# xavi-pinsach/kzg-grandsums-study

Hardware: AMD Instinct MI355X
Metric: grand-sum proofs/sec + MSM G1-adds/sec at n=2^20, 1/2/4/8 MI355X (higher is better)
Workload: dtype u32 limbs (BN254 Fr/Fq Montgomery: 8 x 32-bit; MSM buckets 9 x 29-bit), int VALU; 1 GPU; grandsum prover, n=2^20, k=1, no selectors, inputs resident in HBM; nbits=20, npols=1, selectors=False, parallelism=replicas x1, inflight_per_gpu=4, srs_power=20, srs_points_resident=2097151

## Files before the change

kzg-grandsums-study_amd/csrc/ntt.hip:

```cpp
#include <algorithm>
#include <cstdlib>
#include <map>
#include <mutex>
#include <type_traits>
#include <utility>

#include "fr29.hpp"
#include "kernels.hpp"

namespace kgs {

__device__ __forceinline__ uint32_t bitrev(uint32_t x, int bits) {
  return __builtin_bitreverse32(x) >> (32 - bits);
}

#ifndef KGS_NTT_CANON
__device__ __forceinline__ void bfly_dif(fr& x0, fr& x1, const uint32_t* w, bool tw) {
  const fr a = x0, b = x1;
  x0 = fr::add_lazy(a, b);
  x1 = tw ? fr::mul_nored(fr::sub_2p(a, b), fr::load(w)) : fr::sub_lazy(a, b);
}
__device__ __forceinline__ void bfly_dit(fr& x0, fr& x1, const uint32_t* w, bool tw) {
  const fr a = x0;
  const fr b = tw ? fr::mul_nored(x1, fr::load(w)) : x1;
  x0 = fr::add_lazy(a, b);
  x1 = fr::sub_lazy(a, b);
}
__device__ __forceinline__ fr canon_out(const fr& x) { return x.canon(); }
#else
__device__ __forceinline__ void bfly_dif(fr& x0, fr& x1, const uint32_t* w, bool tw) {
  const fr a = x0, b = x1;
  x0 = a + b;
  fr diff = a - b;
  if (tw) diff = diff * fr::load(w);
  x1 = diff;
}
__device__ __forceinline__ void bfly_dit(fr& x0, fr& x1, const uint32_t* w, bool tw) {
  const fr a = x0;
  fr b = x1;
  if (tw) b = b * fr::load(w);
  x0 = a + b;
  x1 = a - b;
}
__device__ __forceinline__ fr canon_out(const fr& x) { return x; }
#endif


template <int K>
__global__ void __launch_bounds__(256) k_ntt_dif_pass(uint32_t* __restrict__ data,
                                                      const uint32_t* __restrict__ in, uint64_t in_len,
                                                      const uint32_t* __restrict__ pre,
                                                      const uint32_t* __restrict__ tw, int logM, int logm,
                                                      int s0) {
  KGS_AUX_PRIO();
  const uint64_t m = 1ull << logm;
  const uint64_t ngroups = m >> K;
  const uint64_t g = (uint64_t)blockIdx.x * blockDim.x + threadIdx.x;
  if (g >= ngroups) return;
  const int logd = logm - s0 - K;
  const uint64_t d = 1ull << logd;
  const uint64_t lo = g & (d - 1), hi = g >> logd;
  const uint64_t base = (hi << (logd + K)) + lo;
  fr x[1 << K];
#pragma unroll
  for (int r = 0; r < (1 << K); r++) {
    uint64_t idx = base + ((uint64_t)r << logd);
    if (in) {
      if (idx < in_len) {
        x[r] = fr::load(in + 8 * idx);
        if (pre) x[r] = x[r] * fr::load(pre + 8 * idx);
      } else {
        x[r] = fr::zero();
      }
    } else {
      x[r] = fr::load(data + 8 * idx);
    }
  }
#pragma unroll
  for (int k = 0; k < K; k++) {
    const int s = s0 + k;
    const int logh = logm - s - 1;
    const int dist = 1 << (K - 1 - k);
    const uint64_t twbase = 1ull << logh;
#pragma unroll
    for (int j = 0; j < (1 << (K - 1)); j++) {
      const int r = ((j / dist) * 2 * dist) + (j % dist);
      const uint64_t t = lo + ((uint64_t)(j % dist) << logd);
      bfly_dif(x[r], x[r + dist], tw + 8 * (twbase + t), t != 0);
    }
  }
#pragma unroll
  for (int r = 0; r < (1 << K); r++) canon_out(x[r]).store(data + 8 * (base + ((uint64_t)r << logd)));
}

template <int K>
__global__ void __launch_bounds__(256) k_ntt_dit_pass(uint32_t* __restrict__ data,
                                                      const uint32_t* __restrict__ in, int in_bitrev,
                                                      const uint32_t* __restrict__ tw, int logM, int logm,
                                                      int s0, const uint32_t* __restrict__ post,
                                                      const uint32_t* __restrict__ post_s) {
  KGS_AUX_PRIO();
  const uint64_t m = 1ull << logm;
  const uint64_t ngroups = m >> K;
  const uint64_t g = (uint64_t)blockIdx.x * blockDim.x + threadIdx.x;
  if (g >= ngroups) return;
  const int logd = s0;
  const uint64_t d = 1ull << logd;
  const uint64_t lo = g & (d - 1), hi = g >> logd;
  const uint64_t base = (hi << (logd + K)) + lo;
  fr x[1 << K];
#pragma unroll
  for (int r = 0; r < (1 << K); r++) {
    uint64_t idx = base + ((uint64_t)r << logd);
    if (in) {
      uint64_t src = in_bitrev ? idx : (uint64_t)bitrev((uint32_t)idx, logm);
      x[r] = fr::load(in + 8 * src);
    } else {
      x[r] = fr::load(data + 8 * idx);
    }
  }
#pragma unroll
  for (int k = 0; k < K; k++) {
    const int s = s0 + k;
    const int dist = 1 << k;
    const uint64_t twbase = 1ull << s;
#pragma unroll
    for (int j = 0; j < (1 << (K - 1)); j++) {
      const int r = ((j / dist) * 2 * dist) + (j % dist);
      const uint64_t t = lo + ((uint64_t)(j % dist) << logd);
      bfly_dit(x[r], x[r + dist], tw + 8 * (twbase + t), t != 0);
    }
  }
  fr ps;
  if (post_s) ps = fr::load(post_s);
#pragma unroll
  for (int r = 0; r < (1 << K); r++) {
    uint64_t idx = base + ((uint64_t)r << logd);
    fr y = x[r];
    if (post) y = y * fr::load(post + 8 * idx);
    if (post_s) y = y * ps;
    canon_out(y).store(data + 8 * idx);
  }
}

static inline unsigned nblocks(uint64_t work, unsigned bs = 256) { return (unsigned)((work + bs - 1) / bs); }

#ifndef KGS_NTT_ELOG
#define KGS_NTT_ELOG 11
#endif
constexpr int NTT_ELOG = KGS_NTT_ELOG;
constexpr int LDS_ELEMS = 1 << NTT_ELOG;
constexpr int LDS_NT = LDS_ELEMS / 8;

__device__ __forceinline__ void lds_map(uint32_t e, int K, int logd, int lblog, uint32_t& j, uint32_t& cl) {
  if (logd >= lblog) {
    j = e >> lblog;
    cl = e & ((1u << lblog) - 1);
  } else {
    const uint32_t lo = e & ((1u << logd) - 1);
    j = (e >> logd) & ((1u << K) - 1);
    cl = ((e >> (logd + K)) << logd) | lo;
  }
}

__device__ __forceinline__ uint32_t lds_idx(uint32_t col, uint32_t j, int K, int logd) {
  const uint32_t lo = col & ((1u << logd) - 1), hi = col >> logd;
  return (hi << (logd + K)) | (j << logd) | lo;
}

#ifndef KGS_NTT_LDS_AOS
__device__ __forceinline__ uint32_t lds_swz(uint32_t e) { return e ^ ((e >> 4) & 15u) ^ ((e >> 8) & 15u); }
__device__ __forceinline__ fr lds_ld(const uint32_t* lds, uint32_t e) {
  e = lds_swz(e);
  const uint4 a = reinterpret_cast<const uint4*>(lds)[e];
  const uint4 b = reinterpret_cast<const uint4*>(lds + 4 * LDS_ELEMS)[e];
  fr r;
  r.v[0] = a.x; r.v[1] = a.y; r.v[2] = a.z; r.v[3] = a.w;
  r.v[4] = b.x; r.v[5] = b.y; r.v[6] = b.z; r.v[7] = b.w;
  return r;
}
__device__ __forceinline__ void lds_st(uint32_t* lds, uint32_t e, const fr& x) {
  e = lds_swz(e);
  reinterpret_cast<uint4*>(lds)[e] = make_uint4(x.v[0], x.v[1], x.v[2], x.v[3]);
  reinterpret_cast<uint4*>(lds + 4 * LDS_ELEMS)[e] = make_uint4(x.v[4], x.v[5], x.v[6], x.v[7]);
}
#else
__device__ __forceinline__ fr lds_ld(const uint32_t* lds, uint32_t e) { return fr::load(lds + 8 * e); }
__device__ __forceinline__ void lds_st(uint32_t* lds, uint32_t e, const fr& x) { x.store(lds + 8 * e); }
#endif

struct ntt_io {
  uint32_t* data;
  const uint32_t* in;
  uint64_t in_len;
  int in_bitrev;
  const uint32_t* pre;
  const uint32_t* post;
  const uint32_t* post_s;
  int logm;
  const uint32_t* pre29;
  const uint32_t* post29;
  const uint32_t* post_s29;
};

template <bool DIT, bool T29>
__device__ __forceinline__ fr ntt_load(const ntt_io& io, uint64_t idx) {
  if (!io.in) return fr::load(io.data + 8 * idx);
  if (DIT) return fr::load(io.in + 8 * (io.in_bitrev ? idx : (uint64_t)bitrev((uint32_t)idx, io.logm)));
  if (idx >= io.in_len) return fr::zero();
  fr x = fr::load(io.in + 8 * idx);
  if (io.pre) x = T29 ? mul29(x, w29_load(io.pre29 + TW29_WORDS * idx)) : x * fr::load(io.pre + 8 * idx);
  return x;
}
template <bool T29>
__device__ __forceinline__ void ntt_store(const ntt_io& io, uint64_t idx, fr y) {
  if (io.post) y = T29 ? mul29(y, w29_load(io.post29 + TW29_WORDS * idx)) : y * fr::load(io.post + 8 * idx);
  if (io.post_s) y = T29 ? mul29(y, w29_load(io.post_s29)) : y * fr::load(io.post_s);
  canon_out(y).store(io.data + 8 * idx);
}

template <typename TW>
__device__ __forceinline__ TW tw_load(const uint32_t* tw, uint32_t idx);
template <>
__device__ __forceinline__ fr tw_load<fr>(const uint32_t* tw, uint32_t idx) { return fr::load(tw + 8 * idx); }
template <>
__device__ __forceinline__ W29 tw_load<W29>(const uint32_t* tw, uint32_t idx) {
  return w29_load(tw + TW29_WORDS * idx);
}
__device__ __forceinline__ void mul_tw_x2(const fr& a, const fr& wa, const fr& b, const fr& wb, fr& ra, fr& rb) {
  fr::mul_nored_x2(a, wa, b, wb, ra, rb);
}
__device__ __forceinline__ void mul_tw_x2(const fr& a, const W29& wa, const fr& b, const W29& wb, fr& ra, fr& rb) {
  ra = mul29(a, wa);
  rb = mul29(b, wb);
}

template <typename F, int... I>
__device__ __forceinline__ void static_for_impl(F&& f, std::integer_sequence<int, I...>) {
  (f(std::integral_constant<int, I>{}), ...);
}
template <int N, typename F>
__device__ __forceinline__ void static_for(F&& f) {
  static_for_impl(f, std::make_integer_sequence<int, N>{});
}

__device__ __forceinline__ void bfly_pair_triv(fr* x, int r0, int r1, int dist) {
  const fr a0 = x[r0], b0 = x[r0 + dist], a1 = x[r1], b1 = x[r1 + dist];
  x[r0] = fr::add_lazy(a0, b0);
  x[r0 + dist] = fr::sub_lazy(a0, b0);
  x[r1] = fr::add_lazy(a1, b1);
  x[r1 + dist] = fr::sub_lazy(a1, b1);
}
template <bool DIT, typename TW>
__device__ __forceinline__ void bfly_pair_x2(fr* x, int r0, int r1, int dist, const TW& w0, const TW& w1) {
  if (DIT) {
    fr b0, b1;
    mul_tw_x2(x[r0 + dist], w0, x[r1 + dist], w1, b0, b1);
    const fr a0 = x[r0], a1 = x[r1];
    x[r0] = fr::add_lazy(a0, b0);
    x[r0 + dist] = fr::sub_lazy(a0, b0);
    x[r1] = fr::add_lazy(a1, b1);
    x[r1 + dist] = fr::sub_lazy(a1, b1);
  } else {
    const fr d0 = fr::sub_2p(x[r0], x[r0 + dist]), d1 = fr::sub_2p(x[r1], x[r1 + dist]);
    x[r0] = fr::add_lazy(x[r0], x[r0 + dist]);
    x[r1] = fr::add_lazy(x[r1], x[r1 + dist]);
    mul_tw_x2(d0, w0, d1, w1, x[r0 + dist], x[r1 + dist]);
  }
}
template <int R, bool DIT, bool GIN, bool GOUT, bool PF, typename TW>
__device__ __forceinline__ void lds_round(uint32_t* lds, const uint32_t* __restrict__ tw, const ntt_io& io, uint32_t cl,
                                          uint32_t col, uint32_t jb, uint32_t js, int K, int logd, int lb, int kp0) {
  constexpr bool T29 = std::is_same<TW, W29>::value;
  fr x[1 << R];
  if (GIN && !DIT && io.in && io.pre && R >= 2) {
    static_for<(1 << R) / 2>([&](auto rc) {
      constexpr int r = 2 * decltype(rc)::value;
      const uint32_t i0 = lds_idx(col, jb + js * r, K, logd), i1 = lds_idx(col, jb + js * (r + 1), K, logd);
      if (__builtin_expect(__all(i0 >= io.in_len && i1 >= io.in_len), 0)) {
        x[r] = fr::zero();
        x[r + 1] = fr::zero();
        return;
      }
      const fr a0 = i0 < io.in_len ? fr::load(io.in + 8 * i0) : fr::zero();
      const fr a1 = i1 < io.in_len ? fr::load(io.in + 8 * i1) : fr::zero();
      if constexpr (T29) {
        x[r] = mul29(a0, w29_load(io.pre29 + TW29_WORDS * i0));
        x[r + 1] = mul29(a1, w29_load(io.pre29 + TW29_WORDS * i1));
      } else {
        fr::mul_nored_x2(a0, fr::load(io.pre + 8 * i0), a1, fr::load(io.pre + 8 * i1), x[r], x[r + 1]);
      }
    });
  } else {
    static_for<(1 << R)>([&](auto rc) {
      constexpr int r = decltype(rc)::value;
      x[r] = GIN ? ntt_load<DIT, T29>(io, lds_idx(col, jb + js * r, K, logd)) : lds_ld(lds, (jb + js * r) * lb + cl);
    });
  }
#ifdef KGS_NTT_SINGLE
  constexpr bool kPairs = T29;
#else
  constexpr bool kPairs = true;
#endif
  if constexpr (R >= 2 && kPairs) {
    constexpr int half = 1 << (R - 2);
    constexpr int NSTEP = R * half;
    uint32_t tw0[NSTEP], tw1[NSTEP];
    bool triv[NSTEP];
#pragma unroll
    for (int k = 0; k < R; k++) {
      const int kp = kp0 + k;
      const int logh = DIT ? logd + kp : logd + K - 1 - kp;
      const int dist = DIT ? 1 << k : 1 << (R - 1 - k);
      const uint32_t hm = (1u << logh) - 1;
#pragma unroll
      for (int qa = 0; qa < half; qa++) {
        const int r0 = ((qa / dist) * 2 * dist) + (qa % dist), r1 = (((qa + half) / dist) * 2 * dist) + ((qa + half) % dist);
        const uint32_t t0 = lds_idx(col, jb + js * r0, K, logd) & hm, t1 = lds_idx(col, jb + js * r1, K, logd) & hm;
        tw0[k * half + qa] = hm + 1 + t0;
        tw1[k * half + qa] = hm + 1 + t1;
        triv[k * half + qa] = __all(t0 == 0 && t1 == 0);
      }
    }
    TW wa, wb;
    if (PF) {
      wa = tw_load<TW>(tw, tw0[0]);
      wb = tw_load<TW>(tw, tw1[0]);
    }
    static_for<NSTEP>([&](auto stc) {
      constexpr int st = decltype(stc)::value;
      constexpr int k = st / half, qa = st % half;
      constexpr int dist = DIT ? 1 << k : 1 << (R - 1 - k);
      constexpr int r0 = ((qa / dist) * 2 * dist) + (qa % dist), r1 = (((qa + half) / dist) * 2 * dist) + ((qa + half) % dist);
      if (PF) {
        constexpr int nx = st + 1 < NSTEP ? st + 1 : st;
        const TW na = tw_load<TW>(tw, tw0[nx]), nb = tw_load<TW>(tw, tw1[nx]);
        if (triv[st])
          bfly_pair_triv(x, r0, r1, dist);
        else
          bfly_pair_x2<DIT>(x, r0, r1, dist, wa, wb);
        wa = na;
        wb = nb;
      } else if (triv[st]) {
        bfly_pair_triv(x, r0, r1, dist);
      } else {
        bfly_pair_x2<DIT>(x, r0, r1, dist, tw_load<TW>(tw, tw0[st]), tw_load<TW>(tw, tw1[st]));
      }
    });
  } else {
    static_assert(sizeof(TW) == sizeof(fr), "the single-butterfly path reads 8 x 32-bit twiddles only");
#pragma unroll
    for (int k = 0; k < R; k++) {
      const int kp = kp0 + k;
      const int logh = DIT ? logd + kp : logd + K - 1 - kp;
      const int dist = DIT ? 1 << k : 1 << (R - 1 - k);
#pragma unroll
      for (int q = 0; q < (1 << (R - 1)); q++) {
        const int r = ((q / dist) * 2 * dist) + (q % dist);
        const uint32_t idx = lds_idx(col, jb + js * r, K, logd);
        const uint32_t t = idx & ((1u << logh) - 1);
        const uint32_t* w = tw + 8 * ((1u << logh) + t);
        if (DIT)
          bfly_dit(x[r], x[r + dist], w, t != 0);
        else
          bfly_dif(x[r], x[r + dist], w, t != 0);
      }
    }
  }
  if (GOUT && R >= 2) {
    if (io.post) {
      static_for<(1 << R) / 2>([&](auto rc) {
        constexpr int r = 2 * decltype(rc)::value;
        const uint32_t i0 = lds_idx(col, jb + js * r, K, logd), i1 = lds_idx(col, jb + js * (r + 1), K, logd);
        if constexpr (T29) {
          x[r] = mul29(x[r], w29_load(io.post29 + TW29_WORDS * i0));
          x[r + 1] = mul29(x[r + 1], w29_load(io.post29 + TW29_WORDS * i1));
        } else {
          fr::mul_nored_x2_ip(x[r], fr::load(io.post + 8 * i0), x[r + 1], fr::load(io.post + 8 * i1));
        }
      });
    }
    if (io.post_s) {
      if constexpr (T29) {
        const W29 ps = w29_load(io.post_s29);
        static_for<(1 << R)>([&](auto rc) {
          constexpr int r = decltype(rc)::value;
          x[r] = mul29(x[r], ps);
        });
      } else {
        const fr ps = fr::load(io.post_s);
#pragma unroll
        for (int r = 0; r < (1 << R); r += 2) fr::mul_nored_x2_ip(x[r], ps, x[r + 1], ps);
      }
    }
#pragma unroll
    for (int r = 0; r < (1 << R); r++) canon_out(x[r]).store(io.data + 8 * lds_idx(col, jb + js * r, K, logd));
    return;
  }
#pragma unroll
  for (int r = 0; r < (1 << R); r++) {
    if (GOUT)
      ntt_store<T29>(io, lds_idx(col, jb + js * r, K, logd), x[r]);
    else
      lds_st(lds, (jb + js * r) * lb + cl, x[r]);
  }
}

template <int R, bool DIT, bool GIN, bool GOUT, bool PF, typename TW>
__device__ __forceinline__ void lds_round_all(uint32_t* lds, const uint32_t* __restrict__ tw, const ntt_io& io,
                                              uint32_t col0, int K, int logd, int lblog, int b0) {
  const int kp0 = DIT ? b0 : K - b0 - R;
  for (uint32_t g = threadIdx.x; g < (LDS_ELEMS >> R); g += LDS_NT) {
    const uint32_t cl = g & ((1u << lblog) - 1), jq = g >> lblog;
    const uint32_t jb = (jq & ((1u << b0) - 1)) | ((jq >> b0) << (b0 + R));
    lds_round<R, DIT, GIN, GOUT, PF, TW>(lds, tw, io, cl, col0 + cl, jb, 1u << b0, K, logd, 1 << lblog, kp0);
  }
}

#ifndef KGS_NTT_PF3
#define KGS_NTT_PF3 0
#endif
template <int K1, int K2, int K3, int K4, bool DIT, bool DIRECT, int WV, bool T29>
__global__ void __launch_bounds__(LDS_NT) __attribute__((amdgpu_waves_per_eu(WV, WV)))
k_ntt_lds_pass(ntt_io io, const uint32_t* __restrict__ tw, int s0) {
  using TW = typename std::conditional<T29, W29, fr>::type;
  KGS_AUX_PRIO();
  constexpr int K = K1 + K2 + K3 + K4;
  static_assert(K4 == 0 || K3 > 0, "rounds are filled in order");
  constexpr int LBLOG = NTT_ELOG - K;
  constexpr int LB = 1 << LBLOG;
  uint32_t* lds;
  if constexpr (WV >= 3) {
    extern __shared__ __attribute__((aligned(16))) uint32_t lds_dyn[];
    lds = lds_dyn;
  } else {
    __shared__ __attribute__((aligned(16))) uint32_t lds_tile[LDS_ELEMS * 8];
    lds = lds_tile;
  }
  const int logd = DIT ? s0 : io.logm - s0 - K;
  const uint32_t col0 = blockIdx.x * LB;
  if (!DIRECT) {
    for (uint32_t e = threadIdx.x; e < LDS_ELEMS; e += LDS_NT) {
      uint32_t j, cl;
      lds_map(e, K, logd, LBLOG, j, cl);
      lds_st(lds, j * LB + cl, ntt_load<DIT, T29>(io, lds_idx(col0 + cl, j, K, logd)));
    }
    __syncthreads();
  }
  constexpr bool PF = WV < 3 || KGS_NTT_PF3;
  lds_round_all<K1, DIT, DIRECT, false, PF, TW>(lds, tw, io, col0, K, logd, LBLOG, DIT ? 0 : K - K1);
  __syncthreads();
  if constexpr (K4 > 0) {
    lds_round_all<K2, DIT, false, false, PF, TW>(lds, tw, io, col0, K, logd, LBLOG, DIT ? K1 : K3 + K4);
    __syncthreads();
    lds_round_all<K3, DIT, false, false, PF, TW>(lds, tw, io, col0, K, logd, LBLOG, DIT ? K1 + K2 : K4);
    __syncthreads();
    lds_round_all<K4, DIT, false, DIRECT, PF, TW>(lds, tw, io, col0, K, logd, LBLOG, DIT ? K1 + K2 + K3 : 0);
  } else if constexpr (K3 > 0) {
    lds_round_all<K2, DIT, false, false, PF, TW>(lds, tw, io, col0, K, logd, LBLOG, DIT ? K1 : K3);
    __syncthreads();
    lds_round_all<K3, DIT, false, DIRECT, PF, TW>(lds, tw, io, col0, K, logd, LBLOG, DIT ? K1 + K2 : 0);
  } else {
    lds_round_all<K2, DIT, false, DIRECT, PF, TW>(lds, tw, io, col0, K, logd, LBLOG, DIT ? K1 : 0);
  }
  if (!DIRECT) {
    __syncthreads();
    for (uint32_t e = threadIdx.x; e < LDS_ELEMS; e += LDS_NT) {
      uint32_t j, cl;
      lds_map(e, K, logd, LBLOG, j, cl);
      ntt_store<T29>(io, lds_idx(col0 + cl, j, K, logd), lds_ld(lds, j * LB + cl));
    }
  }
}

thread_local bool g_ntt_coresident = false;

struct Tw29Entry {
  uint64_t count;
  const uint32_t* twin;
};
static std::mutex g_tw29_mu;
static std::map<const uint32_t*, Tw29Entry> g_tw29;
void ntt_register_tw29(const uint32_t* base, uint64_t count, const uint32_t* twin) {
  std::lock_guard<std::mutex> lk(g_tw29_mu);
  g_tw29[base] = Tw29Entry{count, twin};
}
void ntt_unregister_tw29(const uint32_t* base) {
  std::lock_guard<std::mutex> lk(g_tw29_mu);
  g_tw29.erase(base);
}
static bool t29_off() {
  static const bool off = [] {
    const char* e = getenv("KGS_NTT_T29");
    return e && e[0] == '0';
  }();
  return off;
}
static const uint32_t* tw29_of(const uint32_t* p) {
  if (!p || t29_off()) return nullptr;
  std::lock_guard<std::mutex> lk(g_tw29_mu);
  auto it = g_tw29.upper_bound(p);
  if (it == g_tw29.begin()) return nullptr;
  --it;
  const uint64_t off = (uint64_t)(p - it->first);
  if (off % 8 || off / 8 >= it->second.count) return nullptr;
  return it->second.twin + (uint64_t)TW29_WORDS * (off / 8);
}

__global__ void k_tw29(uint32_t* __restrict__ out, const uint32_t* __restrict__ in, uint64_t count) {
  const uint64_t i = (uint64_t)blockIdx.x * blockDim.x + threadIdx.x;
  if (i >= count) return;
  fr c;
#pragma unroll
  for (int k = 0; k < 8; k++) c.v[k] = r29::C32[k];
  const fr x = fr::load(in + 8 * i) * c;
  uint32_t l[9];
  unpack29(x, l);
  uint32_t* o = out + (uint64_t)TW29_WORDS * i;
#pragma unroll
  for (int k = 0; k < 9; k++) o[k] = l[k];
  o[9] = 0;
}
void launch_tw29(hipStream_t st, uint32_t* out, const uint32_t* in, uint64_t count) {
  hipLaunchKernelGGL(k_tw29, dim3(nblocks(count)), dim3(256), 0, st, out, in, count);
}

#ifndef KGS_NO_NTT_LDS
constexpr int LDS_MIN_LOGM = NTT_ELOG > 11 ? NTT_ELOG : 11;
constexpr int LDS_MAX_K = NTT_ELOG - 2 < 9 ? NTT_ELOG - 2 : 9;

static int lds_plan(int logm, int* ks) {
  if (NTT_ELOG >= 12) {
    int E = logm < NTT_ELOG ? logm : NTT_ELOG;
    int rest = logm - E;
    if (rest > 0 && rest < 4) {
      E = logm - 4;
      rest = 4;
    }
    const int maxk = NTT_ELOG - 2;
    const int P = 1 + (rest + maxk - 1) / maxk;
    for (int i = 0; i < P - 1; i++) {
      const int left = P - 1 - i;
      ks[i] = (rest + left - 1) / left;
      rest -= ks[i];
    }
    ks[P - 1] = E;
    return P;
  }
  const int P = (logm + LDS_MAX_K - 1) / LDS_MAX_K;
  int E = logm - 6 * (P - 1);
  if (E > LDS_MAX_K) E = LDS_MAX_K;
  int rest = logm - E;
  for (int i = 0; i < P - 1; i++) {
    const int left = P - 1 - i;
    ks[i] = (rest + left - 1) / left;
    rest -= ks[i];
  }
  ks[P - 1] = E;
  return P;
}

static void launch_lds_pass(hipStream_t st, int K, bool dit, uint32_t* data, const uint32_t* in, uint64_t in_len,
                            int in_bitrev, const uint32_t* pre, const uint32_t* tw, int logm, int s0,
                            const uint32_t* post, const uint32_t* post_s) {
  const unsigned blocks = (unsigned)((1ull << logm) / LDS_ELEMS);
  const uint32_t* pre29 = tw29_of(pre);
  const uint32_t* post29 = tw29_of(post);
  const uint32_t* post_s29 = tw29_of(post_s);
  const uint32_t* tw29 = tw29_of(tw);
  if ((pre && !pre29) || (post && !post29) || (post_s && !post_s29)) tw29 = nullptr;
  const ntt_io io{data, in, in_len, in_bitrev, pre, post, post_s, logm, pre29, post29, post_s29};
  const int logd = dit ? s0 : logm - s0 - K;
  static const bool staged = getenv("KGS_NTT_STAGED") != nullptr;
  static const bool direct_tile = getenv("KGS_NTT_DIRECT_TILE") != nullptr;
  const bool direct = logd >= NTT_ELOG - K && (NTT_ELOG - K >= 2 || direct_tile) && !staged;
#define KGS_LDS_LAUNCH2(A, B, C, F, D, E, T, TWP)                                                              \
  do {                                                                                                         \
    if (g_ntt_coresident)                                                                                      \
      hipLaunchKernelGGL((k_ntt_lds_pass<A, B, C, F, D, E, 3, T>), dim3(blocks), dim3(LDS_NT), LDS_ELEMS * 32,  \
                         st, io, TWP, s0);                                                                     \
    else                                                                                                       \
      hipLaunchKernelGGL((k_ntt_lds_pass<A, B, C, F, D, E, 2, T>), dim3(blocks), dim3(LDS_NT), 0, st, io, TWP, \
                         s0);                                                                                  \
  } while (0)
#define KGS_LDS_LAUNCH(A, B, C, F, D, E)             \
  do {                                               \
    if (tw29)                                        \
      KGS_LDS_LAUNCH2(A, B, C, F, D, E, true, tw29); \
    else                                             \
      KGS_LDS_LAUNCH2(A, B, C, F, D, E, false, tw);  \
  } while (0)
#if KGS_NTT_ELOG >= 12
#define KGS_LDS_BY_K_WIDE(D, E)                          \
  case 12: KGS_LDS_LAUNCH(3, 3, 3, 3, D, E); break;      \
  case 11: KGS_LDS_LAUNCH(3, 3, 3, 2, D, E); break;      \
  case 10: KGS_LDS_LAUNCH(3, 3, 2, 2, D, E); break;
#else
#define KGS_LDS_BY_K_WIDE(D, E)
#endif
#define KGS_LDS_BY_K(D, E)                             \
  switch (K) {                                         \
    KGS_LDS_BY_K_WIDE(D, E)                            \
    case 9: KGS_LDS_LAUNCH(3, 3, 3, 0, D, E); break;   \
    case 8: KGS_LDS_LAUNCH(3, 3, 2, 0, D, E); break;   \
    case 7: KGS_LDS_LAUNCH(3, 2, 2, 0, D, E); break;   \
    case 6: KGS_LDS_LAUNCH(3, 3, 0, 0, D, E); break;   \
    case 5: KGS_LDS_LAUNCH(3, 2, 0, 0, D, E); break;   \
    default: KGS_LDS_LAUNCH(2, 2, 0, 0, D, E); break;  \
  }
  if (dit) {
    if (direct) {
      KGS_LDS_BY_K(true, true)
    } else {
      KGS_LDS_BY_K(true, false)
    }
  } else {
    if (direct) {
      KGS_LDS_BY_K(false, true)
    } else {
      KGS_LDS_BY_K(false, false)
    }
  }
#undef KGS_LDS_BY_K
#undef KGS_LDS_BY_K_WIDE
#undef KGS_LDS_LAUNCH
#undef KGS_LDS_LAUNCH2
}
#endif

bool ntt_set_coresident(bool on) {
  const bool prev = g_ntt_coresident;
  g_ntt_coresident = on;
  return prev;
}

void ntt_dif(hipStream_t st, uint32_t* out, const uint32_t* in, uint64_t in_len, int logm,
             const uint32_t* pre, const uint32_t* tw, int logM) {
  if (logm == 0) {
    if (in_len == 0) {
      hipMemsetAsync(out, 0, 32, st);
    } else if (in != out || pre) {
      launch_scale_copy(st, out, in, 1, pre, nullptr);
    }
    return;
  }
#ifndef KGS_NO_NTT_LDS
  if (logm >= LDS_MIN_LOGM) {
    int ks[8];
    const int P = lds_plan(logm, ks);
    for (int i = 0, s0 = 0; i < P; s0 += ks[i++])
      launch_lds_pass(st, ks[i], false, out, i ? nullptr : in, in_len, 1, i ? nullptr : pre, tw, logm, s0, nullptr,
                      nullptr);
    return;
  }
#endif
  int s0 = 0;
  bool first = true;
  while (s0 < logm) {
    const uint32_t* src = first ? in : nullptr;
    const uint32_t* p = first ? pre : nullptr;
    int K = logm - s0 >= 3 ? 3 : logm - s0;
    uint64_t groups = (1ull << logm) >> K;
    if (K == 3)
      hipLaunchKernelGGL(k_ntt_dif_pass<3>, dim3(nblocks(groups)), dim3(256), 0, st, out, src, in_len, p, tw, logM, logm, s0);
    else if (K == 2)
      hipLaunchKernelGGL(k_ntt_dif_pass<2>, dim3(nblocks(groups)), dim3(256), 0, st, out, src, in_len, p, tw, logM, logm, s0);
    else
      hipLaunchKernelGGL(k_ntt_dif_pass<1>, dim3(nblocks(groups)), dim3(256), 0, st, out, src, in_len, p, tw, logM, logm, s0);
    s0 += K;
    first = false;
  }
}

void ntt_dit(hipStream_t st, uint32_t* out, const uint32_t* in, int in_bitrev, int logm,
             const uint32_t* tw, int logM, const uint32_t* post, const uint32_t* post_s) {
  if (logm == 0) {
    launch_scale_copy(st, out, in, 1, post, post_s);
    return;
  }
#ifndef KGS_NO_NTT_LDS
  if (logm >= LDS_MIN_LOGM) {
    int ks[8];
    const int P = lds_plan(logm, ks);
    for (int i = 0, s0 = 0; i < P; i++) {
      const int K = ks[P - 1 - i];
      const bool last = i == P - 1;
      launch_lds_pass(st, K, true, out, i ? nullptr : in, 0, in_bitrev, nullptr, tw, logm, s0, last ? post : nullptr,
                      last ? post_s : nullptr);
      s0 += K;
    }
    return;
  }
#endif
  int rem = logm % 3;
  int s0 = 0;
  bool first = true;
  while (s0 < logm) {
    const uint32_t* src = first ? in : nullptr;
    int K = first && rem ? rem : 3;
    if (K > logm - s0) K = logm - s0;
    uint64_t groups = (1ull << logm) >> K;
    bool last = s0 + K == logm;
    const uint32_t* p = last ? post : nullptr;
    const uint32_t* ps = last ? post_s : nullptr;
    if (K == 3)
      hipLaunchKernelGGL(k_ntt_dit_pass<3>, dim3(nblocks(groups)), dim3(256), 0, st, out, src, in_bitrev, tw, logM, logm, s0, p, ps);
    else if (K == 2)
      hipLaunchKernelGGL(k_ntt_dit_pass<2>, dim3(nblocks(groups)), dim3(256), 0, st, out, src, in_bitrev, tw, logM, logm, s0, p, ps);
    else
      hipLaunchKernelGGL(k_ntt_dit_pass<1>, dim3(nblocks(groups)), dim3(256), 0, st, out, src, in_bitrev, tw, logM, logm, s0, p, ps);
    s0 += K;
    first = false;
  }
}

static void dif_radix(hipStream_t st, uint32_t* data, const uint32_t* tw, int logtotal, int s0, int s1) {
  while (s0 < s1) {
    const int K = s1 - s0 >= 3 ? 3 : s1 - s0;
    const uint64_t groups = (1ull << logtotal) >> K;
    if (K == 3)
      hipLaunchKernelGGL(k_ntt_dif_pass<3>, dim3(nblocks(groups)), dim3(256), 0, st, data, nullptr, 0, nullptr, tw, 0, logtotal, s0);
    else if (K == 2)
      hipLaunchKernelGGL(k_ntt_dif_pass<2>, dim3(nblocks(groups)), dim3(256), 0, st, data, nullptr, 0, nullptr, tw, 0, logtotal, s0);
    else
      hipLaunchKernelGGL(k_ntt_dif_pass<1>, dim3(nblocks(groups)), dim3(256), 0, st, data, nullptr, 0, nullptr, tw, 0, logtotal, s0);
    s0 += K;
  }
}
static void dit_radix(hipStream_t st, uint32_t* data, const uint32_t* tw, int logtotal, int s0, int s1,
                      const uint32_t* post_s) {
  while (s0 < s1) {
    const int K = s1 - s0 >= 3 ? 3 : s1 - s0;
    const uint64_t groups = (1ull << logtotal) >> K;
    const uint32_t* ps = s0 + K == s1 ? post_s : nullptr;
    if (K == 3)
      hipLaunchKernelGGL(k_ntt_dit_pass<3>, dim3(nblocks(groups)), dim3(256), 0, st, data, nullptr, 1, tw, 0, logtotal, s0, nullptr, ps);
    else if (K == 2)
      hipLaunchKernelGGL(k_ntt_dit_pass<2>, dim3(nblocks(groups)), dim3(256), 0, st, data, nullptr, 1, tw, 0, logtotal, s0, nullptr, ps);
    else
      hipLaunchKernelGGL(k_ntt_dit_pass<1>, dim3(nblocks(groups)), dim3(256), 0, st, data, nullptr, 1, tw, 0, logtotal, s0, nullptr, ps);
    s0 += K;
  }
}

void ntt_dif_blocks(hipStream_t st, uint32_t* data, int logtotal, int s, const uint32_t* tw) {
  if (s <= 0) return;
  const int base = logtotal - s;
#ifndef KGS_NO_NTT_LDS
  if (logtotal >= LDS_MIN_LOGM && s >= LDS_MIN_LOGM) {
    int ks[8];
    const int P = lds_plan(s, ks);
    for (int i = 0, s0 = base; i < P; s0 += ks[i++])
      launch_lds_pass(st, ks[i], false, data, nullptr, 0, 1, nullptr, tw, logtotal, s0, nullptr, nullptr);
    return;
  }
  if (logtotal >= LDS_MIN_LOGM && s >= 4) {
    const int K = s < LDS_MAX_K ? s : LDS_MAX_K;
    dif_radix(st, data, tw, logtotal, base, logtotal - K);
    launch_lds_pass(st, K, false, data, nullptr, 0, 1, nullptr, tw, logtotal, logtotal - K, nullptr, nullptr);
    return;
  }
#endif
  dif_radix(st, data, tw, logtotal, base, logtotal);
}

void ntt_dit_blocks(hipStream_t st, uint32_t* data, int logtotal, int s, const uint32_t* tw, const uint32_t* post_s) {
  if (s <= 0) return;
#ifndef KGS_NO_NTT_LDS
  if (logtotal >= LDS_MIN_LOGM && s >= LDS_MIN_LOGM) {
    int ks[8];
    const int P = lds_plan(s, ks);
    for (int i = 0, s0 = 0; i < P; i++) {
      const int K = ks[P - 1 - i];
      launch_lds_pass(st, K, true, data, nullptr, 0, 1, nullptr, tw, logtotal, s0, nullptr, i == P - 1 ? post_s : nullptr);
      s0 += K;
    }
    return;
  }
  if (logtotal >= LDS_MIN_LOGM && s >= 4) {
    const int K = s < LDS_MAX_K ? s : LDS_MAX_K;
    launch_lds_pass(st, K, true, data, nullptr, 0, 1, nullptr, tw, logtotal, 0, nullptr, K == s ? post_s : nullptr);
    dit_radix(st, data, tw, logtotal, K, s, post_s);
    return;
  }
#endif
  dit_radix(st, data, tw, logtotal, 0, s, post_s);
}

__global__ void k_powers(uint32_t* __restrict__ out, uint64_t count, const uint32_t* __restrict__ wp,
                         const uint32_t* __restrict__ scale) {
  KGS_AUX_PRIO();
  const uint64_t t = (uint64_t)blockIdx.x * blockDim.x + threadIdx.x;
  const uint64_t start = t * 64;
  if (start >= count) return;
  fr w = fr::load(wp);
  fr acc = fr::one();
  fr b = w;
  uint64_t e = start;
  while (e) {
    if (e & 1) acc = acc * b;
    b = b.sqr();
    e >>= 1;
  }
  if (scale) acc = acc * fr::load(scale);
  for (uint64_t j = start; j < start + 64 && j < count; j++) {
    acc.store(out + 8 * j);
    acc = acc * w;
  }
}

void launch_powers(hipStream_t st, uint32_t* out, uint64_t count, const uint32_t* w_dev,
                   const uint32_t* scale_dev) {
  uint64_t threads = (count + 63) / 64;
  hipLaunchKernelGGL(k_powers, dim3(nblocks(threads)), dim3(256), 0, st, out, count, w_dev, scale_dev);
}

__global__ void k_scale_copy(uint32_t* __restrict__ out, const uint32_t* __restrict__ in, uint64_t n,
                             const uint32_t* __restrict__ tab, const uint32_t* __restrict__ sc) {
  KGS_AUX_PRIO();
  const uint64_t i = (uint64_t)blockIdx.x * blockDim.x + threadIdx.x;
  if (i >= n) return;
  fr x = fr::load(in + 8 * i);
  if (tab) x = x * fr::load(tab + 8 * i);
  if (sc) x = x * fr::load(sc);
  x.store(out + 8 * i);
}

void launch_scale_copy(hipStream_t st, uint32_t* out, const uint32_t* in, uint64_t n, const uint32_t* tab,
                       const uint32_t* sc) {
  hipLaunchKernelGGL(k_scale_copy, dim3(nblocks(n)), dim3(256), 0, st, out, in, n, tab, sc);
}

__global__ void k_bitrev_copy(uint32_t* __restrict__ out, const uint32_t* __restrict__ in, int logm) {
  KGS_AUX_PRIO();
  const uint64_t i = (uint64_t)blockIdx.x * blockDim.x + threadIdx.x;
  if (i >= (1ull << logm)) return;
  uint64_t j = logm ? bitrev((uint32_t)i, logm) : 0;
  fr::load(in + 8 * j).store(out + 8 * i);
}

void launch_bitrev_copy(hipStream_t st, uint32_t* out, const uint32_t* in, int logm) {
  hipLaunchKernelGGL(k_bitrev_copy, dim3(nblocks(1ull << logm)), dim3(256), 0, st, out, in, logm);
}

}
```

Measured before the change: 97.63 proofs/s.

## Roll repeated NTT LDS rounds into a loop to shrink kernel code size

Restructures the LDS NTT pass so that runs of equal-width rounds execute in a non-unrolled loop, with the global load and store choice passed as runtime flags instead of template parameters. Pre-multiplies are moved to DIF loads only and post-multiplies to DIT stores only. The post-scale sweeps are folded into one loop. The aim is to cut instruction-cache misses caused by large, fully unrolled kernels, as the added code-size and icache profiling scripts suggest. The cost is extra runtime branching, loop overhead and less compile-time specialization in the hot butterfly code.

```diff
diff --git a/kzg-grandsums-study_amd/csrc/ntt.hip b/kzg-grandsums-study_amd/csrc/ntt.hip
--- a/kzg-grandsums-study_amd/csrc/ntt.hip
+++ b/kzg-grandsums-study_amd/csrc/ntt.hip
@@ -203,19 +203,26 @@
   const uint32_t* post_s29;
 };
 
-template <bool DIT, bool T29>
-__device__ __forceinline__ fr ntt_load(const ntt_io& io, uint64_t idx) {
+template <bool DIT>
+__device__ __forceinline__ fr ntt_load_plain(const ntt_io& io, uint64_t idx) {
   if (!io.in) return fr::load(io.data + 8 * idx);
   if (DIT) return fr::load(io.in + 8 * (io.in_bitrev ? idx : (uint64_t)bitrev((uint32_t)idx, io.logm)));
   if (idx >= io.in_len) return fr::zero();
-  fr x = fr::load(io.in + 8 * idx);
-  if (io.pre) x = T29 ? mul29(x, w29_load(io.pre29 + TW29_WORDS * idx)) : x * fr::load(io.pre + 8 * idx);
+  return fr::load(io.in + 8 * idx);
+}
+template <bool DIT, bool T29>
+__device__ __forceinline__ fr ntt_load(const ntt_io& io, uint64_t idx) {
+  fr x = ntt_load_plain<DIT>(io, idx);
+  if (!DIT && io.in && io.pre && idx < io.in_len)
+    x = T29 ? mul29(x, w29_load(io.pre29 + TW29_WORDS * idx)) : x * fr::load(io.pre + 8 * idx);
   return x;
 }
-template <bool T29>
+template <bool DIT, bool T29>
 __device__ __forceinline__ void ntt_store(const ntt_io& io, uint64_t idx, fr y) {
-  if (io.post) y = T29 ? mul29(y, w29_load(io.post29 + TW29_WORDS * idx)) : y * fr::load(io.post + 8 * idx);
-  if (io.post_s) y = T29 ? mul29(y, w29_load(io.post_s29)) : y * fr::load(io.post_s);
+  if (DIT) {
+    if (io.post) y = T29 ? mul29(y, w29_load(io.post29 + TW29_WORDS * idx)) : y * fr::load(io.post + 8 * idx);
+    if (io.post_s) y = T29 ? mul29(y, w29_load(io.post_s29)) : y * fr::load(io.post_s);
+  }
   canon_out(y).store(io.data + 8 * idx);
 }
 
@@ -268,33 +275,42 @@
     mul_tw_x2(d0, w0, d1, w1, x[r0 + dist], x[r1 + dist]);
   }
 }
-template <int R, bool DIT, bool GIN, bool GOUT, bool PF, typename TW>
+template <int R, bool DIT, bool MAYGIN, bool MAYGOUT, bool PF, typename TW>
 __device__ __forceinline__ void lds_round(uint32_t* lds, const uint32_t* __restrict__ tw, const ntt_io& io, uint32_t cl,
-                                          uint32_t col, uint32_t jb, uint32_t js, int K, int logd, int lb, int kp0) {
+                                          uint32_t col, uint32_t jb, uint32_t js, int K, int logd, int lb, int kp0,
+                                          bool gin, bool gout) {
   constexpr bool T29 = std::is_same<TW, W29>::value;
+  static_assert(R >= 2, "rounds of at least two stages: the products go two at a time");
   fr x[1 << R];
-  if (GIN && !DIT && io.in && io.pre && R >= 2) {
-    static_for<(1 << R) / 2>([&](auto rc) {
-      constexpr int r = 2 * decltype(rc)::value;
-      const uint32_t i0 = lds_idx(col, jb + js * r, K, logd), i1 = lds_idx(col, jb + js * (r + 1), K, logd);
-      if (__builtin_expect(__all(i0 >= io.in_len && i1 >= io.in_len), 0)) {
-        x[r] = fr::zero();
-        x[r + 1] = fr::zero();
-        return;
-      }
-      const fr a0 = i0 < io.in_len ? fr::load(io.in + 8 * i0) : fr::zero();
-      const fr a1 = i1 < io.in_len ? fr::load(io.in + 8 * i1) : fr::zero();
-      if constexpr (T29) {
-        x[r] = mul29(a0, w29_load(io.pre29 + TW29_WORDS * i0));
-        x[r + 1] = mul29(a1, w29_load(io.pre29 + TW29_WORDS * i1));
-      } else {
-        fr::mul_nored_x2(a0, fr::load(io.pre + 8 * i0), a1, fr::load(io.pre + 8 * i1), x[r], x[r + 1]);
-      }
-    });
+  if (MAYGIN && gin) {
+    if (!DIT && io.in && io.pre) {
+      static_for<(1 << R) / 2>([&](auto rc) {
+        constexpr int r = 2 * decltype(rc)::value;
+        const uint32_t i0 = lds_idx(col, jb + js * r, K, logd), i1 = lds_idx(col, jb + js * (r + 1), K, logd);
+        if (__builtin_expect(__all(i0 >= io.in_len && i1 >= io.in_len), 0)) {
+          x[r] = fr::zero();
+          x[r + 1] = fr::zero();
+          return;
+        }
+        const fr a0 = i0 < io.in_len ? fr::load(io.in + 8 * i0) : fr::zero();
+        const fr a1 = i1 < io.in_len ? fr::load(io.in + 8 * i1) : fr::zero();
+        if constexpr (T29) {
+          x[r] = mul29(a0, w29_load(io.pre29 + TW29_WORDS * i0));
+          x[r + 1] = mul29(a1, w29_load(io.pre29 + TW29_WORDS * i1));
+        } else {
+          fr::mul_nored_x2(a0, fr::load(io.pre + 8 * i0), a1, fr::load(io.pre + 8 * i1), x[r], x[r + 1]);
+        }
+      });
+    } else {
+      static_for<(1 << R)>([&](auto rc) {
+        constexpr int r = decltype(rc)::value;
+        x[r] = ntt_load_plain<DIT>(io, lds_idx(col, jb + js * r, K, logd));
+      });
+    }
   } else {
     static_for<(1 << R)>([&](auto rc) {
       constexpr int r = decltype(rc)::value;
-      x[r] = GIN ? ntt_load<DIT, T29>(io, lds_idx(col, jb + js * r, K, logd)) : lds_ld(lds, (jb + js * r) * lb + cl);
+      x[r] = lds_ld(lds, (jb + js * r) * lb + cl);
     });
   }
 #ifdef KGS_NTT_SINGLE
@@ -302,7 +318,7 @@
 #else
   constexpr bool kPairs = true;
 #endif
-  if constexpr (R >= 2 && kPairs) {
+  if constexpr (kPairs) {
     constexpr int half = 1 << (R - 2);
     constexpr int NSTEP = R * half;
     uint32_t tw0[NSTEP], tw1[NSTEP];
@@ -332,7 +348,7 @@
       constexpr int k = st / half, qa = st % half;
       constexpr int dist = DIT ? 1 << k : 1 << (R - 1 - k);
       constexpr int r0 = ((qa / dist) * 2 * dist) + (qa % dist), r1 = (((qa + half) / dist) * 2 * dist) + ((qa + half) % dist);
-      if (PF) {
+      if constexpr (PF) {
         constexpr int nx = st + 1 < NSTEP ? st + 1 : st;
         const TW na = tw_load<TW>(tw, tw0[nx]), nb = tw_load<TW>(tw, tw1[nx]);
         if (triv[st])
@@ -348,7 +364,7 @@
       }
     });
   } else {
-    static_assert(sizeof(TW) == sizeof(fr), "the single-butterfly path reads 8 x 32-bit twiddles only");
+    static_assert(kPairs || sizeof(TW) == sizeof(fr), "the single-butterfly path reads 8 x 32-bit twiddles only");
 #pragma unroll
     for (int k = 0; k < R; k++) {
       const int kp = kp0 + k;
@@ -367,53 +383,61 @@
       }
     }
   }
-  if (GOUT && R >= 2) {
-    if (io.post) {
-      static_for<(1 << R) / 2>([&](auto rc) {
-        constexpr int r = 2 * decltype(rc)::value;
-        const uint32_t i0 = lds_idx(col, jb + js * r, K, logd), i1 = lds_idx(col, jb + js * (r + 1), K, logd);
+  if (MAYGOUT && gout) {
+    if constexpr (DIT) {
+      const int nsweep = (io.post != nullptr) + (io.post_s != nullptr);
+#pragma unroll 1
+      for (int sw = 0; sw < nsweep; sw++) {
+        const bool tab = io.post != nullptr && sw == 0;
         if constexpr (T29) {
-          x[r] = mul29(x[r], w29_load(io.post29 + TW29_WORDS * i0));
-          x[r + 1] = mul29(x[r + 1], w29_load(io.post29 + TW29_WORDS * i1));
+          const uint32_t* rec = tab ? io.post29 : io.post_s29;
+          const uint32_t stride = tab ? TW29_WORDS : 0;
+          static_for<(1 << R)>([&](auto rc) {
+            constexpr int r = decltype(rc)::value;
+            x[r] = mul29(x[r], w29_load(rec + (uint64_t)stride * lds_idx(col, jb + js * r, K, logd)));
+          });
         } else {
-          fr::mul_nored_x2_ip(x[r], fr::load(io.post + 8 * i0), x[r + 1], fr::load(io.post + 8 * i1));
+          const uint32_t* rec = tab ? io.post : io.post_s;
+          const uint32_t stride = tab ? 8 : 0;
+          static_for<(1 << R) / 2>([&](auto rc) {
+            constexpr int r = 2 * decltype(rc)::value;
+            const uint32_t i0 = lds_idx(col, jb + js * r, K, logd), i1 = lds_idx(col, jb + js * (r + 1), K, logd);
+            fr::mul_nored_x2_ip(x[r], fr::load(rec + (uint64_t)stride * i0), x[r + 1], fr::load(rec + (uint64_t)stride * i1));
+          });
         }
-      });
-    }
-    if (io.post_s) {
-      if constexpr (T29) {
-        const W29 ps = w29_load(io.post_s29);
-        static_for<(1 << R)>([&](auto rc) {
-          constexpr int r = decltype(rc)::value;
-          x[r] = mul29(x[r], ps);
-        });
-      } else {
-        const fr ps = fr::load(io.post_s);
-#pragma unroll
-        for (int r = 0; r < (1 << R); r += 2) fr::mul_nored_x2_ip(x[r], ps, x[r + 1], ps);
       }
     }
-#pragma unroll
-    for (int r = 0; r < (1 << R); r++) canon_out(x[r]).store(io.data + 8 * lds_idx(col, jb + js * r, K, logd));
-    return;
-  }
-#pragma unroll
-  for (int r = 0; r < (1 << R); r++) {
-    if (GOUT)
-      ntt_store<T29>(io, lds_idx(col, jb + js * r, K, logd), x[r]);
-    else
+    static_for<(1 << R)>([&](auto rc) {
+      constexpr int r = decltype(rc)::value;
+      canon_out(x[r]).store(io.data + 8 * lds_idx(col, jb + js * r, K, logd));
+    });
+  } else {
+    static_for<(1 << R)>([&](auto rc) {
+      constexpr int r = decltype(rc)::value;
       lds_st(lds, (jb + js * r) * lb + cl, x[r]);
-  }
-}
-
-template <int R, bool DIT, bool GIN, bool GOUT, bool PF, typename TW>
-__device__ __forceinline__ void lds_round_all(uint32_t* lds, const uint32_t* __restrict__ tw, const ntt_io& io,
-                                              uint32_t col0, int K, int logd, int lblog, int b0) {
-  const int kp0 = DIT ? b0 : K - b0 - R;
-  for (uint32_t g = threadIdx.x; g < (LDS_ELEMS >> R); g += LDS_NT) {
-    const uint32_t cl = g & ((1u << lblog) - 1), jq = g >> lblog;
-    const uint32_t jb = (jq & ((1u << b0) - 1)) | ((jq >> b0) << (b0 + R));
-    lds_round<R, DIT, GIN, GOUT, PF, TW>(lds, tw, io, cl, col0 + cl, jb, 1u << b0, K, logd, 1 << lblog, kp0);
+    });
+  }
+}
+
+template <int R, int NR, bool DIT, bool DIRECT, bool FIRST, bool LAST, bool PF, typename TW>
+__device__ __forceinline__ void lds_rounds(uint32_t* lds, const uint32_t* __restrict__ tw, const ntt_io& io,
+                                           uint32_t col0, int K, int logd, int lblog, int bfirst) {
+  constexpr bool MAYGIN = DIRECT && FIRST, MAYGOUT = DIRECT && LAST;
+#pragma unroll 1
+  for (int i = 0; i < NR; i++) {
+    int iv = i;
+    if (NR > 1) asm volatile("" : "+s"(iv));
+    const int b0 = DIT ? bfirst + R * iv : bfirst - R * iv;
+    const int kp0 = DIT ? b0 : K - b0 - R;
+    const bool gin = MAYGIN && iv == 0, gout = MAYGOUT && iv == NR - 1;
+#pragma unroll 1
+    for (uint32_t g = threadIdx.x; g < (LDS_ELEMS >> R); g += LDS_NT) {
+      const uint32_t cl = g & ((1u << lblog) - 1), jq = g >> lblog;
+      const uint32_t jb = (jq & ((1u << b0) - 1)) | ((jq >> b0) << (b0 + R));
+      lds_round<R, DIT, MAYGIN, MAYGOUT, PF, TW>(lds, tw, io, cl, col0 + cl, jb, 1u << b0, K, logd, 1 << lblog, kp0,
+                                                 gin, gout);
+    }
+    if (!MAYGOUT || iv != NR - 1) __syncthreads();
   }
 }
 
@@ -427,6 +451,11 @@
   KGS_AUX_PRIO();
   constexpr int K = K1 + K2 + K3 + K4;
   static_assert(K4 == 0 || K3 > 0, "rounds are filled in order");
+  constexpr int N1 = 1 + (K2 == K1) + (K2 == K1 && K3 == K1) + (K2 == K1 && K3 == K1 && K4 == K1);
+  constexpr int RB = N1 == 1 ? K2 : N1 == 2 ? K3 : N1 == 3 ? K4 : 0;
+  constexpr int N2 = RB == 0 ? 0 : (K - N1 * K1) / RB;
+  static_assert(N1 * K1 + N2 * RB == K, "a plan is a run of K1-stage rounds and a run of narrower ones");
+  static_assert(N1 + N2 >= 2, "at least two rounds");
   constexpr int LBLOG = NTT_ELOG - K;
   constexpr int LB = 1 << LBLOG;
   uint32_t* lds;
@@ -440,6 +469,7 @@
   const int logd = DIT ? s0 : io.logm - s0 - K;
   const uint32_t col0 = blockIdx.x * LB;
   if (!DIRECT) {
+#pragma unroll 1
     for (uint32_t e = threadIdx.x; e < LDS_ELEMS; e += LDS_NT) {
       uint32_t j, cl;
       lds_map(e, K, logd, LBLOG, j, cl);
@@ -448,27 +478,32 @@
     __syncthreads();
   }
   constexpr bool PF = WV < 3 || KGS_NTT_PF3;
-  lds_round_all<K1, DIT, DIRECT, false, PF, TW>(lds, tw, io, col0, K, logd, LBLOG, DIT ? 0 : K - K1);
-  __syncthreads();
-  if constexpr (K4 > 0) {
-    lds_round_all<K2, DIT, false, false, PF, TW>(lds, tw, io, col0, K, logd, LBLOG, DIT ? K1 : K3 + K4);
-    __syncthreads();
-    lds_round_all<K3, DIT, false, false, PF, TW>(lds, tw, io, col0, K, logd, LBLOG, DIT ? K1 + K2 : K4);
-    __syncthreads();
-    lds_round_all<K4, DIT, false, DIRECT, PF, TW>(lds, tw, io, col0, K, logd, LBLOG, DIT ? K1 + K2 + K3 : 0);
-  } else if constexpr (K3 > 0) {
-    lds_round_all<K2, DIT, false, false, PF, TW>(lds, tw, io, col0, K, logd, LBLOG, DIT ? K1 : K3);
-    __syncthreads();
-    lds_round_all<K3, DIT, false, DIRECT, PF, TW>(lds, tw, io, col0, K, logd, LBLOG, DIT ? K1 + K2 : 0);
+  constexpr bool ROLLED = T29 || WV < 3 || DIT;
+  if constexpr (ROLLED) {
+    lds_rounds<K1, N1, DIT, DIRECT, true, N2 == 0, PF, TW>(lds, tw, io, col0, K, logd, LBLOG, DIT ? 0 : K - K1);
+    if constexpr (N2 > 0)
+      lds_rounds<RB, N2, DIT, DIRECT, false, true, PF, TW>(lds, tw, io, col0, K, logd, LBLOG,
+                                                           DIT ? N1 * K1 : K - N1 * K1 - RB);
   } else {
-    lds_round_all<K2, DIT, false, DIRECT, PF, TW>(lds, tw, io, col0, K, logd, LBLOG, DIT ? K1 : 0);
+    lds_rounds<K1, 1, DIT, DIRECT, true, false, PF, TW>(lds, tw, io, col0, K, logd, LBLOG, DIT ? 0 : K - K1);
+    if constexpr (K3 > 0) {
+      lds_rounds<K2, 1, DIT, DIRECT, false, false, PF, TW>(lds, tw, io, col0, K, logd, LBLOG, DIT ? K1 : K3 + K4);
+      if constexpr (K4 > 0) {
+        lds_rounds<K3, 1, DIT, DIRECT, false, false, PF, TW>(lds, tw, io, col0, K, logd, LBLOG, DIT ? K1 + K2 : K4);
+        lds_rounds<K4, 1, DIT, DIRECT, false, true, PF, TW>(lds, tw, io, col0, K, logd, LBLOG, DIT ? K1 + K2 + K3 : 0);
+      } else {
+        lds_rounds<K3, 1, DIT, DIRECT, false, true, PF, TW>(lds, tw, io, col0, K, logd, LBLOG, DIT ? K1 + K2 : 0);
+      }
+    } else {
+      lds_rounds<K2, 1, DIT, DIRECT, false, true, PF, TW>(lds, tw, io, col0, K, logd, LBLOG, DIT ? K1 : 0);
+    }
   }
   if (!DIRECT) {
-    __syncthreads();
+#pragma unroll 1
     for (uint32_t e = threadIdx.x; e < LDS_ELEMS; e += LDS_NT) {
       uint32_t j, cl;
       lds_map(e, K, logd, LBLOG, j, cl);
-      ntt_store<T29>(io, lds_idx(col0 + cl, j, K, logd), lds_ld(lds, j * LB + cl));
+      ntt_store<DIT, T29>(io, lds_idx(col0 + cl, j, K, logd), lds_ld(lds, j * LB + cl));
     }
   }
 }
diff --git a/profiles/code_size.py b/profiles/code_size.py
--- /dev/null
+++ b/profiles/code_size.py
@@ -0,0 +1,114 @@
+#!/usr/bin/env python3
+import argparse
+import os
+import shutil
+import struct
+import subprocess
+import sys
+
+ROOT = os.path.dirname(os.path.dirname(os.path.abspath(__file__)))
+MAGIC = b"__CLANG_OFFLOAD_BUNDLE__"
+PROOF_2P20 = [
+    "kgs::k_accumulate<3,", "kgs::k_sort_part<17,", "kgs::k_sort_hist<17,", "kgs::k_lo_scatter", "kgs::k_combine(",
+    "kgs::k_quotient<false, false>", "kgs::k_rowcol16", "kgs::k_div_finish", "kgs::k_builder_finish<false, false>",
+    "kgs::k_eval_tiles", "kgs::k_lincomb", "kgs::k_builder_tileprod<false, false>", "kgs::k_divcheck<false, false>",
+    "kgs::k_to_mont", "kgs::k_lo_count", "kgs::k_bitsum_rc", "kgs::k_sort_scan_blocks", "kgs::k_apply_carry<false>",
+    "kgs::k_div_carries", "kgs::k_tile_inverse", "kgs::k_degree", "kgs::k_combine_level", "kgs::k_tile_carry<false>",
+    "kgs::k_sort_scan(",
+    "kgs::k_ntt_lds_pass<3, 3, 0, 0, false, true, 3, true>", "kgs::k_ntt_lds_pass<3, 3, 0, 0, true, true, 3, true>",
+    "kgs::k_ntt_lds_pass<3, 3, 3, 0, false, false, 3, true>", "kgs::k_ntt_lds_pass<3, 3, 2, 0, true, false, 3, true>",
+    "kgs::k_ntt_lds_pass<3, 3, 3, 0, true, false, 3, true>",
+]
+
+
+def short(name):
+    name = name[5:] if name.startswith("void ") else name
+    return name.split("(")[0] + "("
+
+
+def in_proof(name):
+    return any(short(name).startswith(p) for p in PROOF_2P20)
+
+
+def code_objects(blob, arch):
+    out, pos = [], 0
+    while True:
+        pos = blob.find(MAGIC, pos)
+        if pos < 0:
+            return out
+        n = struct.unpack_from("<Q", blob, pos + len(MAGIC))[0]
+        p = pos + len(MAGIC) + 8
+        if n > 64:
+            pos += len(MAGIC)
+            continue
+        for _ in range(n):
+            off, size, tlen = struct.unpack_from("<QQQ", blob, p)
+            triple = blob[p + 24:p + 24 + tlen].decode()
+            p += 24 + tlen
+            if triple.startswith("hip") and triple.endswith(arch) and size:
+                out.append(blob[pos + off:pos + off + size])
+        pos += len(MAGIC)
+
+
+def kernel_sizes(elf):
+    assert elf[:4] == b"\x7fELF" and elf[4] == 2, "not an ELF64 code object"
+    shoff = struct.unpack_from("<Q", elf, 0x28)[0]
+    shentsize, shnum = struct.unpack_from("<HH", elf, 0x3A)
+    sec = [struct.unpack_from("<IIQQQQIIQQ", elf, shoff + i * shentsize) for i in range(shnum)]
+    funcs, kds = {}, set()
+    for s in sec:
+        if s[1] != 2:
+            continue
+        stroff = sec[s[6]][4]
+        for i in range(s[5] // 24):
+            name, info, _, _, _, size = struct.unpack_from("<IBBHQQ", elf, s[4] + 24 * i)
+            end = elf.index(b"\0", stroff + name)
+            sym = elf[stroff + name:end].decode()
+            if sym.endswith(".kd"):
+                kds.add(sym[:-3])
+            elif info & 15 == 2:
+                funcs[sym] = size
+    return {k: v for k, v in funcs.items() if k in kds}
+
+
+def demangle(names):
+    filt = shutil.which("llvm-cxxfilt") or shutil.which("c++filt")
+    if filt is None:
+        return list(names)
+    out = subprocess.run([filt], input="\n".join(names), capture_output=True, text=True, check=True).stdout
+    return out.rstrip("\n").split("\n")
+
+
+def table(lib, arch="gfx950"):
+    with open(lib, "rb") as fh:
+        blob = fh.read()
+    sizes = {}
+    for co in code_objects(blob, arch):
+        sizes.update(kernel_sizes(co))
+    if not sizes:
+        sys.exit(f"{lib}: no {arch} code object found (a compressed bundle?)")
+    syms = sorted(sizes)
+    return sorted(((sizes[s], d) for s, d in zip(syms, demangle(syms))), key=lambda r: (-r[0], r[1]))
+
+
+def main():
+    ap = argparse.ArgumentParser()
+    ap.add_argument("lib", nargs="?", default=os.path.join(ROOT, "kzg-grandsums-study_amd", "lib", "libkgs.so"))
+    ap.add_argument("--arch", default="gfx950")
+    ap.add_argument("--min", type=int, default=0, help="list kernels of at least this many bytes")
+    ap.add_argument("--cache", type=int, default=65536)
+    args = ap.parse_args()
+    rows = table(args.lib, args.arch)
+    print(f"code bytes per kernel, {args.arch}; * = launched by a 2^20 grand-sum proof, > = above {args.cache} B")
+    for size, name in rows:
+        if size < args.min:
+            continue
+        mark = ("*" if in_proof(name) else " ") + (">" if size > args.cache else " ")
+        print(f"{size:8d} {mark} {short(name)[:-1]}")
+    hot = [(s, n) for s, n in rows if in_proof(n)]
+    print(f"{len(rows)} kernels, {sum(s for s, _ in rows)} B; of the 2^20 proof: {len(hot)} kernels, "
+          f"{sum(s for s, _ in hot)} B, {sum(1 for s, _ in hot if s > args.cache)} above {args.cache} B")
+
+
+if __name__ == "__main__":
+    main()
diff --git a/profiles/summarize_icache.py b/profiles/summarize_icache.py
--- /dev/null
+++ b/profiles/summarize_icache.py
@@ -0,0 +1,33 @@
+#!/usr/bin/env python3
+import collections
+import csv
+import sys
+
+
+def totals(path):
+    tot = collections.defaultdict(collections.Counter)
+    for r in csv.DictReader(open(path)):
+        name = r["Kernel_Name"].split("(")[0].replace("kgs::", "").replace("void ", "")
+        tot[name][r["Counter_Name"]] += float(r["Counter_Value"])
+        tot[name]["dispatches:" + r["Counter_Name"]] += 1
+    return tot
+
+
+def ratio(a, b):
+    return f"{a / b:8.4f}" if b else "       -"
+
+
+def main():
+    a = totals(sys.argv[1])
+    b = totals(sys.argv[2]) if len(sys.argv) > 2 else {}
+    print("   req M   miss M  missrate  fetchlat  wait/wave  winst/wave    VALU M  calls  kernel")
+    for k in sorted(a, key=lambda k: -a[k]["SQC_ICACHE_REQ"]):
+        ca, cb = a[k], b.get(k, collections.Counter())
+        print(f"{ca['SQC_ICACHE_REQ'] / 1e6:8.2f} {ca['SQC_ICACHE_MISSES'] / 1e6:8.3f}  "
+              f"{ratio(ca['SQC_ICACHE_MISSES'], ca['SQC_ICACHE_REQ'])}  {ratio(ca['SQ_IFETCH_LEVEL'], ca['SQ_IFETCH'])}   "
+              f"{ratio(cb['SQ_WAIT_ANY'], cb['SQ_WAVE_CYCLES'])}    {ratio(cb['SQ_WAIT_INST_ANY'], cb['SQ_WAVE_CYCLES'])} "
+              f"{cb['SQ_INSTS_VALU'] / 1e6:9.2f} {int(ca['dispatches:SQC_ICACHE_REQ']):6d}  {k}")
+
+
+if __name__ == "__main__":
+    main()
```

Result: no change. 97.39 proofs/s (-0.2%).
